# iamsonderr/icl-mixed-precision-gmres

Measured on AMD Instinct MI355X. Metric: GMRES iterations/sec + SpMV achieved HBM GB/s, 10M-nnz CSR, 1/2/4/8 GPUs, higher is better.
Workload: dtype f32; 1 GPU; BAND banded CSR n=1000000, offsets -5..+4, nnz=9999975 (1e6 rows = 10M nnz per GPU, 1 GPU(s)); GMRES(30) mixed (fp32 Arnoldi, f32 accumulation, fp64 residual/update), cgs, identity preconditioner, tol=0; step=one restart cycle = 30 iterations, rows_per_gpu=1000000, nnz=9999975, parallelism=one GPU

## Files before the change

### icl-mixed-precision-gmres_amd/__init__.py

```python
from __future__ import annotations

import ctypes as C
import os
import subprocess
from dataclasses import dataclass, field
from pathlib import Path
from typing import Optional

import numpy as np

from ._abi import (ACCUMS, ENGINES, MODES, ORTHS, PRECS, SPMV_FORMATS, STATUS, CondestResult, HostCsr, RankLayout, SolveArgs, SolveResult,
                   condest_args, condest_dict)

PKG_DIR = Path(__file__).resolve().parent
REPO_DIR = PKG_DIR.parent
LIB_DIR = PKG_DIR / "lib"
HIP_LIB = LIB_DIR / "libmpgmres_hip.so"
HOST_LIB = LIB_DIR / "libmpgmres_host.so"
CLI = PKG_DIR / "bin" / "gmres_perf_test"


def build(jobs: int = 8) -> None:
    subprocess.run(["make", "-C", str(PKG_DIR), f"-j{jobs}"], check=True)

# ... 132 lines not shown
    lib.mpg_halo_local_cols.argtypes = [C.c_void_p, P32]
    lib.mpg_halo_free.argtypes = [C.c_void_p]
    lib.mpg_halo_free.restype = None
    lib.mpg_rccl_unique_id.argtypes = [C.c_char_p, C.c_int]
    lib.mpg_engine_create_dist.argtypes = [C.POINTER(SolveArgs), C.c_void_p, C.c_char_p, _I32, _I32,
                                           C.POINTER(C.c_void_p), C.c_char_p, C.c_int]
    lib.mpg_solve_loopback.argtypes = [C.POINTER(SolveArgs), _I32, C.POINTER(SolveResult)]
    lib.mpg_solve_loopback_ex.argtypes = [C.POINTER(SolveArgs), _I32, C.POINTER(SolveResult), C.c_void_p]
    lib.mpg_solve_multi_gpu.argtypes = [C.POINTER(SolveArgs), _I32, C.c_void_p, C.POINTER(SolveResult), C.c_void_p]
    lib.mpg_engine_comm_ranks.argtypes = [C.c_void_p]
    lib.mpg_engine_sell_columns.argtypes = [C.c_void_p, C.POINTER(C.c_int32), C.POINTER(C.c_int64),
                                            C.POINTER(C.c_int64)]
    lib.mpg_engine_half_stats.argtypes = [C.c_void_p, C.POINTER(C.c_int64)]
    lib.mpg_engine_slices_per_wave.argtypes = [C.c_void_p]
    lib.mpg_engine_givens_folded.argtypes = [C.c_void_p]
    lib.mpg_engine_accum.argtypes = [C.c_void_p]
    lib.mpg_engine_prologue_format.argtypes = [C.c_void_p]
    lib.mpg_engine_sell_shared_slices.argtypes = [C.c_void_p]
    lib.mpg_engine_sell_shared_slices.restype = C.c_int64
    lib.mpg_engine_sell_sigma.argtypes = [C.c_void_p]


_HIP_DECLS = {
    "mpg_error_string": ([C.c_int], C.c_char_p),
    "mpg_ctx_last_error": ([_P], C.c_char_p),
    "mpg_ctx_create": ([C.c_int, C.POINTER(_P)], C.c_int),
    "mpg_ctx_destroy": ([_P], C.c_int),
    "mpg_ctx_sync": ([_P], C.c_int),
    "mpg_ctx_stream": ([_P], _P),
    "mpg_malloc": ([_P, C.c_size_t, C.POINTER(_P)], C.c_int),
# ... 578 lines not shown
        per = (C.c_double * cap)()
        which = {"spmv": 0, "cgs_update": 2, "dots": 3}[phase]
        cnt = self._lib.mpg_engine_time_phase_stamps(self._h, which, reps, C.byref(ms), per, cap)
        if cnt < 0:
            msg = self._lib.mpg_engine_last_error(self._h).decode(errors="replace")
            raise RuntimeError(f"mpg_engine_time_phase_stamps failed ({cnt}): {msg}")
        return ms.value, [per[i] for i in range(min(cnt, cap))]

    def phase_bytes(self, phase: str) -> float:
        return float(self._lib.mpg_engine_phase_bytes(self._h, self.PHASES[phase]))

    def spmv_layout(self) -> dict:
        f, w, cb, st, win = C.c_int32(), C.c_int32(), C.c_int32(), C.c_int64(), C.c_int32()
        if self._lib.mpg_engine_spmv_layout(self._h, C.byref(f), C.byref(w), C.byref(cb), C.byref(st), C.byref(win)):
            raise RuntimeError("mpg_engine_spmv_layout failed")
        return {"format": {1: "csr", 2: "sell", 3: "node"}[f.value], "vec_width": w.value, "col_bytes": cb.value,
                "stored": st.value, "window": bool(win.value),
                "slices_per_wave": int(self._lib.mpg_engine_slices_per_wave(self._h)),
                "givens_folded": bool(self._lib.mpg_engine_givens_folded(self._h) == 1),
                "accum": {0: "f64", 1: "f32"}[int(self._lib.mpg_engine_accum(self._h))],
                "prologue": {1: "csr", 2: "sell", 3: "node"}[int(self._lib.mpg_engine_prologue_format(self._h))]}

    def sell_columns(self) -> dict:
        f, e, i = C.c_int32(), C.c_int64(), C.c_int64()
        if self._lib.mpg_engine_sell_columns(self._h, C.byref(f), C.byref(e), C.byref(i)):
            raise RuntimeError("mpg_engine_sell_columns failed")
        return {"form": {-1: "none", 0: "int32", 1: "int16", 2: "stepped"}[f.value], "csr_slices": e.value,
                "implicit_slices": i.value,
                "shared_slices": int(self._lib.mpg_engine_sell_shared_slices(self._h)),
                "sigma": int(self._lib.mpg_engine_sell_sigma(self._h))}

    def comm_ranks(self) -> int:
        return int(self._lib.mpg_engine_comm_ranks(self._h))

    def half_stats(self) -> dict:
        st = (C.c_int64 * 4)()
# ... 15 lines not shown
```

### icl-mixed-precision-gmres_amd/csrc/arnoldi.hip

```cpp
#include "arnoldi_kernels.hpp"
#include "arnoldi_launch.hpp"

#include <cstdlib>
#include <new>
#include <algorithm>
#include <vector>

using namespace mpg;

namespace {

int64_t sell_copy_bytes(const mpg_arnoldi* a);

void node_prologue_build(mpg_arnoldi* a) {
    const char* e = std::getenv("MPG_NODE_PROLOGUE");
    if ((e && *e == '0') || a->node.nblk == 0 || a->d.n_front != 0 || a->d.outer_type != MPG_F64) return;
    if (hipMalloc((void**)&a->rsum, (size_t)std::max(a->d.n, 1) * sizeof(double)) != hipSuccess) {
        (void)hipGetLastError();
        return;
    }
    if (a->d.val_outer == a->d.val_inner && a->d.inner_val == MPG_F64) {
        a->node_res = &a->node;
        return;
    }
// ... 288 lines not shown
    });
    if (st) return st;
    MPG_LAUNCH_CHECK(a->ctx);
    return MPG_OK;
}

int mpg_arnoldi_reduce(mpg_arnoldi_t a, int ncols) {
    return a && a->acc32 ? mpg_acc32::reduce(a, ncols) : reduce_run<double>(a, ncols);
}

int mpg_arnoldi_spmv(mpg_arnoldi_t a, int k) { return spmv_impl(a, k, 0); }
int mpg_arnoldi_spmv_dots(mpg_arnoldi_t a, int k, int fold) {
    if (fold < 0 || fold > 2) return MPG_ERR_ARG;
    return spmv_impl(a, k, fold, true);
}
int mpg_arnoldi_givens_spmv(mpg_arnoldi_t a, int k) { return spmv_impl(a, k, 1); }
int mpg_arnoldi_givens_partials_spmv(mpg_arnoldi_t a, int k) { return spmv_impl(a, k, 2); }
int mpg_arnoldi_fold_max_m(void) { return kFoldMaxM; }
int mpg_arnoldi_partials_max_cols(void) { return kWideMax; }

constexpr int kFoldMaxGroups = 4096;
int mpg_arnoldi_fold_pays(mpg_arnoldi_t a) {
    if (!a) return 0;
    const char* env = std::getenv("MPG_FOLD_MAX_GROUPS");
    const int64_t limit = env && *env ? std::atoll(env) : kFoldMaxGroups;
    if (a->node.nblk > 0) {
        const int tpw = node_tpw(a->node);
        return (a->node.ntiles + tpw - 1) / tpw <= limit ? 1 : 0;
    }
    const SellCopy& S = a->sell;
// ... 78 lines not shown
```

### icl-mixed-precision-gmres_amd/csrc/arnoldi_acc32.hip

```cpp
#include "arnoldi_launch.hpp"

namespace mpg_acc32 {
int reduce(mpg_arnoldi* a, int ncols) { return reduce_run<float>(a, ncols); }
int spmv(mpg_arnoldi* a, int k, int fold, bool dots) { return spmv_run<float>(a, k, fold, dots); }
int dots(mpg_arnoldi* a, int k, bool combine) { return dots_run<float>(a, k, combine); }
int cgs(mpg_arnoldi* a, int k, int pass, bool givens, bool from_partials, bool no_next) {
    return cgs_run<float>(a, k, pass, givens, from_partials, no_next);
}
int mgs(mpg_arnoldi* a, int k, int j, bool from_partials) { return mgs_run<float>(a, k, j, from_partials); }
int givens(mpg_arnoldi* a, int k, bool from_partials) { return givens_run<float>(a, k, from_partials); }
int update(mpg_arnoldi* a, int k) { return update_run<float>(a, k); }
}
```

### icl-mixed-precision-gmres_amd/csrc/arnoldi_kernels.hpp

```cpp
#pragma once

#include "csr_tile.hpp"
#include "node_tile.hpp"
#include "sell_tile.hpp"
#include "handoff.hpp"
#include "panel.hpp"
#include "internal.hpp"
#include "mpgmres/arnoldi.h"

#include <cstdlib>
#include <new>
#include <algorithm>
#include <vector>

using namespace mpg;

namespace {

constexpr int kNC = 32;
constexpr int kGroups = 1024;
constexpr int kCombineBlock = 1024;
constexpr int kCombineGroups = 256;
constexpr int kOrthMGS = 1, kOrthCGSR = 2;

// ... 854 lines not shown
            }
        }
    }
    for (int i = n4 + blockIdx.x * BS + threadIdx.x; i < n; i += gridDim.x * BS) {
        const A wi = (A)w[i];
#pragma unroll
        for (int c = 0; c < kNC; ++c)
            if (c < nc) acc[c] += (A)Vb[(int64_t)c * ld + i] * wi;
    }
    store_partials<kNC, BS, COMBINE>(acc, nc, partial + (size_t)c0 * gridDim.x);
    if constexpr (COMBINE) {
        if (last_arriver(cnt)) combine_columns<BS, A>(partial, gridDim.x, nc, sums);
    }
}

template <class T, int BS, int NC, class A = double>
__device__ __forceinline__ void dots_panel(int n, const T* __restrict__ V, int64_t ld, const T* __restrict__ w,
                                           double* __restrict__ partial) {
    static_assert(NC >= 1 && NC <= kNC, "one panel");
    constexpr int NP = Pow2Ceil<NC>::v;
    constexpr int B = kColBatch<T>;
    A acc[NP];
#pragma unroll
    for (int c = 0; c < NP; ++c) acc[c] = A(0);
    const int n4 = n & ~3;
    for (int i = 4 * (blockIdx.x * BS + threadIdx.x); i < n4; i += 4 * gridDim.x * BS) {
        A wv[4];
        Row4<T>::load(w + i, wv);
#pragma unroll
        for (int c0 = 0; c0 < NC; c0 += B) {
            Raw4<T> v[B];
#pragma unroll
            for (int u = 0; u < B; ++u)
                if (c0 + u < NC) v[u].load(V + (int64_t)(c0 + u) * ld + i);
            __builtin_amdgcn_sched_barrier(0);
#pragma unroll
            for (int u = 0; u < B; ++u)
                if (c0 + u < NC)
                    acc[c0 + u] += v[u].template at<A>(0) * wv[0] + v[u].template at<A>(1) * wv[1] +
                                   v[u].template at<A>(2) * wv[2] + v[u].template at<A>(3) * wv[3];
            asm volatile("" : "+v"(acc[c0]) : : "memory");
        }
    }
    for (int i = n4 + blockIdx.x * BS + threadIdx.x; i < n; i += gridDim.x * BS) {
        const A wi = (A)w[i];
#pragma unroll
        for (int c = 0; c < NC; ++c) acc[c] += (A)V[(int64_t)c * ld + i] * wi;
    }
    store_partials<NP, BS>(acc, NC, partial);
}

template <class T, int BS, int NC, bool STAMP = false, class A = double>
__global__ __launch_bounds__(BS) void k_dots_nc(int n, const T* __restrict__ V, int64_t ld,
                                                const T* __restrict__ w, double* __restrict__ partial,
                                                unsigned long long* stamp) {
    stamp_at<STAMP>(stamp, 0);
    dots_panel<T, BS, NC, A>(n, V, ld, w, partial);
    stamp_at<STAMP>(stamp, 1);
}

template <class T, int BS, int NCL, class A = double>
__global__ __launch_bounds__(BS) void k_dots_panels(int n, const T* __restrict__ V, int64_t ld,
                                                    const T* __restrict__ w, double* __restrict__ partial) {
    const int c0 = blockIdx.y * kNC;
    double* __restrict__ part = partial + (size_t)c0 * gridDim.x;
    if (blockIdx.y + 1 < gridDim.y) dots_panel<T, BS, kNC, A>(n, V + (int64_t)c0 * ld, ld, w, part);
    else dots_panel<T, BS, NCL, A>(n, V + (int64_t)c0 * ld, ld, w, part);
}

template <class T, int BS, int NC, bool FROM_PARTS = false, bool NEXT_DOTS = false, bool PF = false,
          bool STAMP = false, class A = double>
__global__ __launch_bounds__(BS) void k_cgs_update_nc(int n, const T* __restrict__ V, int64_t ld,
                                                      const double* __restrict__ sums, int part_G,
// ... 587 lines not shown
    double* dpart = nullptr;
    double* sums = nullptr;
    double* report = nullptr;
    unsigned* counters = nullptr;
    int Gd = 1;
    SellCopy sell;
    SellCopy sell_outer;
    NodeCopy node;
    NodeCopy node_outer;
    const NodeCopy* node_res = nullptr;
    double* rsum = nullptr;
    bool outer_is_inner = false;
    double* fd_part = nullptr;
    unsigned* fd_cnt = nullptr;
    int fd_gs = 0, fd_ng = 0;
    bool acc32 = false;

    char* small_at(int slot) const { return static_cast<char*>(small) + (size_t)slot * (d.m + 1) * tsize; }
    void* cs() const { return small_at(0); }
    void* sn() const { return small_at(1); }
    void* s() const { return small_at(2); }
    void* corr() const { return small_at(3); }
    void* inv() const { return small_at(4); }
};

namespace {

int combo_of(const mpg_arnoldi_desc& d) {
    if (d.vec_type == MPG_F64 && d.outer_type == MPG_F64 && d.inner_val == MPG_F64)
        return d.prec_type == MPG_F64 ? 0 : (d.prec_type == MPG_F32 ? 1 : -1);
// ... 50 lines not shown
```

### icl-mixed-precision-gmres_amd/csrc/arnoldi_launch.hpp

```cpp
#pragma once

#include "arnoldi_kernels.hpp"

#include <algorithm>
#include <cstdlib>
#include <type_traits>

namespace {

template <class A, class F>
int dispatch_acc(int combo, F&& f) {
    if constexpr (std::is_same_v<A, double>) {
        return dispatch(combo, f);
    } else {
        switch (combo) {
            case 2: return f(float(), float(), float(), float());
            case 3: return f(float(), double(), float(), float());
            case 4: return f(float(), double(), float(), half_v());
            default: return MPG_ERR_UNSUPPORTED;
        }
    }
}

template <class A>
// ... 142 lines not shown
            Acsr->blocks, Acsr->nblocks, Acsr->rowptr, Acsr->col, static_cast<const VI*>(a->d.val_inner), Acsr->nnz,
            static_cast<const T*>(a->w[k & 1]), static_cast<const T*>(a->inv()), static_cast<T*>(a->V), a->ld, k,
            diag, static_cast<T*>(a->w[(k + 1) & 1]), gf, a->d.inner_row_exp);
        return (int)MPG_OK;
    });
    if (st) return st;
    if (dots) {
        a->last_G = a->fd_ng;
        a->last_part = a->dpart;
    }
    MPG_LAUNCH_CHECK(a->ctx);
    return MPG_OK;
}


inline int wide_groups(const mpg_arnoldi* a, int ncols) {
    const int np = (ncols + kNC - 1) / kNC;
    return std::max(1, std::min(a->Gd, kCombineGroups / np));
}

inline unsigned long long* take_stamp(mpg_arnoldi* a, int64_t waves) {
    unsigned long long* p = a->ctx->stamp_next;
    a->ctx->stamp_next = nullptr;
    return p && waves <= a->ctx->stamp_cap ? p : nullptr;
}

template <class A>
int dots_run(mpg_arnoldi_t a, int k, bool combine) {
    if (!a || k < 0 || k >= a->d.m) return MPG_ERR_ARG;
    const int ndots_all = a->d.orth == kOrthMGS ? 1 : k + 1;
// ... 206 lines not shown
                static_cast<X*>(a->d.x));
        }
        return (int)MPG_OK;
    });
    if (st) return st;
    MPG_LAUNCH_CHECK(a->ctx);
    return MPG_OK;
}


}

namespace mpg_acc32 {
int reduce(mpg_arnoldi* a, int ncols);
int spmv(mpg_arnoldi* a, int k, int fold, bool dots);
int dots(mpg_arnoldi* a, int k, bool combine);
int cgs(mpg_arnoldi* a, int k, int pass, bool givens, bool from_partials, bool no_next);
int mgs(mpg_arnoldi* a, int k, int j, bool from_partials);
int givens(mpg_arnoldi* a, int k, bool from_partials);
int update(mpg_arnoldi* a, int k);
}
```

### icl-mixed-precision-gmres_amd/host/fused_gmres.cpp

```cpp
#include "fused_gmres.hpp"

#include <algorithm>
#include <chrono>
#include <cmath>
#include <cstdio>
#include <cstring>
#include <functional>
#include <stdexcept>
#include <thread>

#include "gmres.hpp"
#include "types_hip.hpp"

namespace mpg {

DevMem::DevMem(mpg_ctx_t c, size_t b) : ctx(c), bytes(b) { check(mpg_malloc(c, b, &p), "mpg_malloc", c); }
DevMem::~DevMem() {
    if (p) mpg_free(ctx, p);
}
DevMem& DevMem::operator=(DevMem&& o) noexcept {
    if (this != &o) {
        if (p) mpg_free(ctx, p);
        ctx = o.ctx;
        p = o.p;
// ... 37 lines not shown
    std::function<double(size_t)> step_loss;
    LostOrthogonalityFused(double tol, double restart_tol, size_t m, size_t max_restarts)
        : Base(tol, m, max_restarts), restart_tol_squared_(restart_tol * restart_tol) {}
    iteration_action check_initial(double r, double nrm, double pr, double pb) override {
        current_loss_squared_ = 0;
        return Base::check_initial(r, nrm, pr, pb);
    }
    iteration_action check(size_t k, double res, double bnorm) override {
        const iteration_action a = Base::check(k, res, bnorm);
        if (a != iteration_next) return a;
        current_loss_squared_ += step_loss(k);
        return current_loss_squared_ >= restart_tol_squared_ ? iteration_restart : iteration_next;
    }
    bool needs_arnoldi_residual() const override { return true; }
};

}

struct FusedEngine::Impl {
    mpg_ctx_t ctx = nullptr;
    mpg_solve_args args{};
    Comm* comm = nullptr;
    ModeTypes ty{};
    int n = 0, n_ext = 0, m = 0, orth = 0;
    int front = 0;
    void* xp = nullptr;
    int64_t nnz = 0;
    DevMem rowptr, col, val64, val_outer_own, val_inner_own, diag, b, x, tmp_t, tmp_p, scal;
    DevMem row_exp;
    int64_t half_stats[4] = {0, 0, 0, 0};
// ... 4 lines not shown
    double* rep[2] = {nullptr, nullptr};
    double* report_host = nullptr;
    int report_len = 0;
    bool pipeline = true;
    DevMem x_snap;
    hipEvent_t report_ev[2] = {nullptr, nullptr};
    hipGraph_t graph = nullptr;
    hipGraphExec_t graph_exec = nullptr;
    bool use_graph = true;
    bool fold = false;
    bool combine = false;
    bool cgs_partials = false;
    bool fuse_dots = false;
    bool fuse_dots_required = false;
    int fuse_dots_k0 = 32;
    int timed = -1;
    bool timed_inplace = false;
    bool timed_graph = false;
    std::vector<hipEvent_t> marks;
    unsigned long long* stamps = nullptr;
    int dup_phase = -1;
    int64_t dup_count = 0;
    int64_t dup_with_dots = 0;
    int64_t stamp_cap = 0, stamp_q = 0, stamp_max = 0;
    std::vector<int32_t> rowptr_host;
    mpg_ilu_t ilu = nullptr;
    bool orthloss = false;
    DevMem loss_S, loss_u;

    ~Impl() {
// ... 222 lines not shown
    conv_->total_iters = 0;
    breakdown.stop = a.stop_on_breakdown != 0;

    const char* env = std::getenv("MPG_NO_GRAPH");
    I.use_graph = !(env && *env == '1') && (!comm || comm->capturable());
    const char* cenv = std::getenv("MPG_COMBINE");
    I.combine = !comm && cenv && *cenv == '1' && I.orth != MPG_ORTH_MGS && I.m <= mpg_arnoldi_fold_max_m();
    const char* penv = std::getenv("MPG_CGS_PARTIALS");
    I.cgs_partials = !I.combine && I.orth != MPG_ORTH_MGS &&
                     (I.orth == MPG_ORTH_CGSR ? (penv && *penv == '1') : !(penv && *penv == '0'));
    const char* denv = std::getenv("MPG_FUSE_DOTS");
    I.fuse_dots = I.cgs_partials && I.orth == MPG_ORTH_CGS && denv && (*denv == '1' || *denv == '2');
    I.fuse_dots_required = I.fuse_dots && *denv == '2';
    const char* kenv = std::getenv("MPG_FUSE_DOTS_K0");
    I.fuse_dots_k0 = kenv && *kenv ? std::max(0, std::min(32, std::atoi(kenv))) : 32;
    const char* fenv = std::getenv("MPG_FOLD_GIVENS");
    bool fold_on = fenv && *fenv ? *fenv != '0' : mpg_arnoldi_fold_pays(I.arn) != 0;
    if (comm && !(fenv && *fenv)) {
        double* flag = I.scal.as<double>() + 6;
        const double no = fold_on ? 0.0 : 1.0;
        check(mpg_memcpy_h2d(ctx, flag, &no, sizeof no), "h2d", ctx);
        comm->allreduce_max(flag, 1, I.stream());
        double any_no = 0;
        check(mpg_memcpy_d2h(ctx, &any_no, flag, sizeof any_no), "d2h", ctx);
        fold_on = any_no == 0.0;
    }
    I.fold = !I.combine && fold_on && I.m <= mpg_arnoldi_fold_max_m();
    check(mpg_ctx_sync(ctx), "sync", ctx);
    setup_seconds = std::chrono::duration<double>(clk::now() - t0).count();
    prologue();
// ... 47 lines not shown

void FusedEngine::step(int k, bool fold) {
    Impl& I = *p_;
    if (I.fuse_dots && !I.comm && !I.ilu && I.orth == MPG_ORTH_CGS && I.cgs_partials && !I.combine &&
        k + 1 <= I.fuse_dots_k0) {
        timed(0, [&] { check(mpg_arnoldi_spmv(I.arn, k), "spmv", I.ctx); });
        const int st = mpg_arnoldi_spmv_dots(I.arn, k, fold && k > 0 ? 2 : 0);
        timed_end(0);
        if (st == MPG_OK) {
            check(mpg_arnoldi_cgs_partials(I.arn, k), "cgs", I.ctx);
            if (!fold) givens(k);
            return;
        }
        if (st != MPG_ERR_UNSUPPORTED || I.fuse_dots_required) check(st, "spmv+dots", I.ctx);
        I.fuse_dots = false;
    }
    if (fold && k > 0) {
        if (I.comm)
            I.comm->allreduce_sum_and_halo(mpg_arnoldi_partials_dev(I.arn), mpg_arnoldi_partials_count(I.arn),
                                           mpg_arnoldi_wprev_dev(I.arn, k), mpg_arnoldi_vec_bytes(I.arn),
                                           I.stream());
        timed(0, [&] { check(mpg_arnoldi_spmv(I.arn, k), "spmv", I.ctx); });
        check(mpg_arnoldi_givens_partials_spmv(I.arn, k), "givens+spmv", I.ctx);
        dup(0, [&] { check(mpg_arnoldi_givens_partials_spmv(I.arn, k), "givens+spmv", I.ctx); });
        timed_end(0);
    } else {
        if (I.comm) I.comm->halo(mpg_arnoldi_wprev_dev(I.arn, k), mpg_arnoldi_vec_bytes(I.arn), I.stream());
        timed(0, [&] { check(mpg_arnoldi_spmv(I.arn, k), "spmv", I.ctx); });
        check(mpg_arnoldi_spmv(I.arn, k), "spmv", I.ctx);
        dup(0, [&] { check(mpg_arnoldi_spmv(I.arn, k), "spmv", I.ctx); });
// ... 365 lines not shown
}

double FusedEngine::phase_bytes(int which) const {
    const Impl& I = *p_;
    const double n = I.n, z = (double)I.nnz, sT = (double)dsize(I.ty.T), sX = (double)dsize(I.ty.X);
    const double sV = (double)dsize(I.ty.VI), sP = (double)dsize(I.ty.P);
    const double jac = I.args.prec == MPG_PREC_JACOBI ? 1.0 : 0.0;
    if (which == 0) {
        return z * (sV + 4) + (n + 1) * 4 + 2 * n * sT + jac * n * sP;
    }
    if (which == 1) return z * (sX + 4) + (n + 1) * 4 + 3 * n * sX + n * sT + jac * n * sP;
    if (which == 4) {
        int32_t fmt = 0, W = 0, cb = 0, win = 0;
        int64_t stored = 0;
        check(mpg_arnoldi_spmv_layout(I.arn, &fmt, &W, &cb, &stored, &win), "layout", I.ctx);
        const double vec = 3 * n * sT + jac * n * sP;
        if (fmt == 2 || fmt == 3) return (double)mpg_arnoldi_sell_matrix_bytes(I.arn) + vec;
        return z * (sV + 4) + (n + 1) * 4 + vec;
    }
    if (which == 3) {
        double cols = 0;
        for (int k = 0; k < I.m; ++k) cols += (I.orth == MPG_ORTH_MGS ? 1 : k + 1);
        return (cols / I.m + 1) * n * sT;
    }
    return ((I.m - 1) / 2.0 + 1) * n * sT + 2 * n * sT;
}

mpg_arnoldi_t FusedEngine::arnoldi() const { return p_->arn; }
const int64_t* FusedEngine::half_stats() const { return p_->half_stats; }
bool FusedEngine::givens_folded() const { return p_->fold; }

constexpr int kTimedReplays = 10;

double FusedEngine::time_phase(int which, int reps, bool inplace, std::vector<double>* per_launch) {
    measured = true;
    Impl& I = *p_;
    if (inplace && which != 0) throw std::invalid_argument("in-place timing covers the Arnoldi SpMV only");
    I.timed = which;
    I.timed_inplace = inplace;
    I.marks.clear();
    for (int r = 0; r < reps; ++r) cycle_program();
    I.timed = -1;
    I.timed_inplace = false;
    hipck(hipStreamSynchronize(I.stream()), "sync");
    float total_ms = 0;
// ... 194 lines not shown
    cleanup();
    if (!count) throw StatusError(MPG_ERR_UNSUPPORTED, "no launch of the phase stored stamps");
    return total / count;
}

double FusedEngine::time_phase_dup(int which, int reps, int64_t* launches) {
    measured = true;
    Impl& I = *p_;
    if (!I.use_graph) throw StatusError(MPG_ERR_UNSUPPORTED, "the cycle is not captured (MPG_NO_GRAPH / eager ranks)");
    if (which != 0 && which != 2 && which != 3) throw std::invalid_argument("phase: 0 spmv, 2 cgs update, 3 dots");
    hipGraph_t g[2] = {nullptr, nullptr};
    hipGraphExec_t ge[2] = {nullptr, nullptr};
    hipEvent_t ev[2] = {nullptr, nullptr};
    auto cleanup = [&] {
        I.dup_phase = -1;
        for (int q = 0; q < 2; ++q) {
            if (ge[q]) (void)hipGraphExecDestroy(ge[q]);
            if (g[q]) (void)hipGraphDestroy(g[q]);
            if (ev[q]) (void)hipEventDestroy(ev[q]);
        }
    };
    std::vector<double> diff;
    int64_t added = 0, with_dots = 0;
    try {
        for (int q = 0; q < 2; ++q) {
            I.dup_phase = q ? which : -1;
            I.dup_count = 0;
            I.dup_with_dots = 0;
            hipck(hipStreamBeginCapture(I.stream(), hipStreamCaptureModeThreadLocal), "begin capture");
            try {
                cycle_program();
            } catch (...) {
                (void)hipStreamEndCapture(I.stream(), &g[q]);
                throw;
            }
            hipck(hipStreamEndCapture(I.stream(), &g[q]), "end capture");
            hipck(hipGraphInstantiate(&ge[q], g[q], nullptr, nullptr, 0), "instantiate");
            if (q) {
                added = I.dup_count;
                with_dots = I.dup_with_dots;
            }
        }
        I.dup_phase = -1;
        if (added < 1) throw StatusError(MPG_ERR_UNSUPPORTED, "the cycle has no launch of that phase");
        for (hipEvent_t& e : ev) hipck(hipEventCreate(&e), "event");
        for (int q = 0; q < 2; ++q) hipck(hipGraphLaunch(ge[q], I.stream()), "graph launch");
        hipck(hipStreamSynchronize(I.stream()), "sync");
        for (int r = 0; r < reps; ++r) {
            float ms[2] = {0, 0};
            for (int q = 0; q < 2; ++q) {
                hipck(hipEventRecord(ev[0], I.stream()), "record");
                hipck(hipGraphLaunch(ge[q], I.stream()), "graph launch");
                hipck(hipEventRecord(ev[1], I.stream()), "record");
                hipck(hipEventSynchronize(ev[1]), "sync");
                hipck(hipEventElapsedTime(&ms[q], ev[0], ev[1]), "elapsed");
            }
            diff.push_back((double)(ms[1] - ms[0]) / (double)added);
        }
    } catch (...) {
        cleanup();
        (void)hipGetLastError();
        throw;
    }
    cleanup();
    if (launches) *launches = added;
    std::sort(diff.begin(), diff.end());
    double ms = diff[diff.size() / 2];
    if (with_dots) ms -= time_phase_dup(3, reps) * (double)with_dots / (double)added;
    return ms;
}

void fill_history(const FusedEngine& e, mpg_solve_result* r) {
    r->status = e.status;
    r->restarts = e.restarts;
    r->inner_k = e.inner_k;
    r->total_iters = (int64_t)e.total_iters();
    r->minvb_norm = e.minvb_norm;
    r->setup_seconds = e.setup_seconds;
    r->n_cycles = (int64_t)e.cycles.size();
    for (size_t c = 0; c < e.cycles.size() && (int64_t)c < r->cycle_cap; ++c) {
        if (r->cyc_r_norm) r->cyc_r_norm[c] = e.cycles[c].r_norm;
        if (r->cyc_normalization) r->cyc_normalization[c] = e.cycles[c].normalization;
        if (r->cyc_beta) r->cyc_beta[c] = e.cycles[c].beta;
// ... 194 lines not shown
int mpg_engine_accum(mpg_engine_t e) {
    if (!e || !e->eng) return MPG_ERR_ARG;
    return mpg_arnoldi_accum(e->eng->arnoldi());
}

int mpg_engine_prologue_format(mpg_engine_t e) {
    if (!e || !e->eng) return MPG_ERR_ARG;
    return mpg_arnoldi_prologue_format(e->eng->arnoldi());
}

int mpg_engine_givens_folded(mpg_engine_t e) {
    if (!e || !e->eng) return MPG_ERR_ARG;
    return e->eng->givens_folded() ? 1 : 0;
}

int mpg_engine_comm_ranks(mpg_engine_t e) {
    if (!e || !e->eng) return MPG_ERR_ARG;
    return e->comm ? e->comm->transport_ranks() : 1;
}

int64_t mpg_engine_sell_shared_slices(mpg_engine_t e) {
    if (!e || !e->eng) return MPG_ERR_ARG;
    return mpg_arnoldi_sell_shared_slices(e->eng->arnoldi());
}

int mpg_engine_sell_sigma(mpg_engine_t e) {
    if (!e || !e->eng) return MPG_ERR_ARG;
    return mpg_arnoldi_sell_sigma(e->eng->arnoldi());
}

// ... 27 lines not shown
```

### icl-mixed-precision-gmres_amd/host/fused_gmres.hpp

```cpp
#ifndef MPGMRES_FUSED_GMRES_HPP
#define MPGMRES_FUSED_GMRES_HPP

#include <hip/hip_runtime.h>

#include <memory>
#include <string>
#include <vector>

#include "IterUtil.hpp"
#include "mpgmres/arnoldi.h"
#include "mpgmres/capi.h"
#include "mpgmres/solve.h"

namespace mpg {

class Comm {
public:
    virtual ~Comm() {}
    virtual int size() const = 0;
    virtual int rank() const = 0;
    virtual void allreduce_sum(double* dev, int count, hipStream_t s) = 0;
    virtual void allreduce_max(double* dev, int count, hipStream_t s) = 0;
    virtual void halo(void* dev_vec, int elem_bytes, hipStream_t s) = 0;
    virtual void allreduce_sum_and_halo(double* dev, int count, void* dev_vec, int elem_bytes, hipStream_t s) {
// ... 27 lines not shown
    FusedEngine(mpg_ctx_t ctx, const mpg_solve_args& args, Comm* comm = nullptr, int n_ext = -1, int n_front = 0);
    ~FusedEngine();

    int run(int max_cycles, bool& done);
    void finish_report(mpg_solve_result* r);

    size_t total_iters() const { return conv_->total_iterations(); }
    double time_phase(int which, int reps, bool inplace = false, std::vector<double>* per_launch = nullptr);
    double time_phase_graph(int which, int reps, std::vector<double>* per_launch = nullptr);
    double time_phase_stamps(int which, int reps, std::vector<double>* per_launch = nullptr);
    double time_phase_dup(int which, int reps, int64_t* launches = nullptr);
    double phase_bytes(int which) const;
    mpg_arnoldi_t arnoldi() const;
    const int64_t* half_stats() const;
    bool givens_folded() const;
    void sync();

    std::vector<CycleRecord> cycles;
    std::vector<double> step_res;
    std::vector<int> step_cycle;
    int status = 0;
    int64_t restarts = 0;
    int64_t inner_k = 0;
    double minvb_norm = 0, b_norm = 0, a_norm = 0;
    double setup_seconds = 0;
    BreakdownLog breakdown;
    bool measured = false;

private:
    struct Impl;
// ... 39 lines not shown
```

### include/mpgmres/arnoldi.h

```cpp
#ifndef MPGMRES_ARNOLDI_H
#define MPGMRES_ARNOLDI_H

#include <stdint.h>

#include "mpgmres/capi.h"

#ifdef __cplusplus
extern "C" {
#endif

typedef enum { MPG_F64 = 0, MPG_F32 = 1, MPG_F16 = 2 } mpg_dtype_t;

typedef struct mpg_arnoldi* mpg_arnoldi_t;

typedef struct {
    int32_t n;
    int32_t n_ext;
    int32_t m;
    int32_t orth;
    int32_t vec_type;
    int32_t outer_type;
    int32_t prec_type;
    int32_t inner_val;
    int32_t jacobi;
// ... 28 lines not shown
int mpg_arnoldi_spmv(mpg_arnoldi_t a, int k);
int mpg_arnoldi_dots(mpg_arnoldi_t a, int k);
int mpg_arnoldi_cgs(mpg_arnoldi_t a, int k, int pass);
int mpg_arnoldi_cgs_partials(mpg_arnoldi_t a, int k);
int mpg_arnoldi_partials_max_cols(void);
int mpg_arnoldi_cgsr_wide_pass(mpg_arnoldi_t a, int k, int pass);
int mpg_arnoldi_mgs(mpg_arnoldi_t a, int k, int j);
int mpg_arnoldi_mgs_partials(mpg_arnoldi_t a, int k, int j);
int mpg_arnoldi_givens(mpg_arnoldi_t a, int k);
int mpg_arnoldi_givens_partials(mpg_arnoldi_t a, int k);
int mpg_arnoldi_givens_spmv(mpg_arnoldi_t a, int k);
int mpg_arnoldi_dots_sums(mpg_arnoldi_t a, int k);
int mpg_arnoldi_cgs_givens(mpg_arnoldi_t a, int k, int pass);
int mpg_arnoldi_givens_partials_spmv(mpg_arnoldi_t a, int k);
int mpg_arnoldi_spmv_dots(mpg_arnoldi_t a, int k, int fold);
int mpg_arnoldi_fold_max_m(void);
int mpg_arnoldi_fold_pays(mpg_arnoldi_t a);
int mpg_arnoldi_update(mpg_arnoldi_t a, int k);
int mpg_arnoldi_reduce(mpg_arnoldi_t a, int ncols);

double* mpg_arnoldi_sums_dev(mpg_arnoldi_t a);
void* mpg_arnoldi_wprev_dev(mpg_arnoldi_t a, int k);
int mpg_arnoldi_vec_bytes(mpg_arnoldi_t a);
const double* mpg_arnoldi_report_dev(mpg_arnoldi_t a);
int mpg_arnoldi_report_len(mpg_arnoldi_t a);
const void* mpg_arnoldi_basis_dev(mpg_arnoldi_t a, int64_t* ld);
const void* mpg_arnoldi_hessenberg_dev(mpg_arnoldi_t a);
const void* mpg_arnoldi_inv_dev(mpg_arnoldi_t a);
int mpg_arnoldi_time_next_spmv(mpg_arnoldi_t a, void* start_event, void* stop_event);
int mpg_arnoldi_stamp_next(mpg_arnoldi_t a, unsigned long long* slots, int64_t cap_waves);
// ... 20 lines not shown
```

### include/mpgmres/solve.h

```cpp
#ifndef MPGMRES_SOLVE_H
#define MPGMRES_SOLVE_H

#include <stddef.h>
#include <stdint.h>

#ifdef __cplusplus
extern "C" {
#endif

typedef enum {
    MPG_MODE_MIXED = 0,
    MPG_MODE_BASELINE = 1,
    MPG_MODE_SINGLE_PREC = 2,
    MPG_MODE_SINGLE = 3,
    MPG_MODE_MIXED_HALF = 4
} mpg_mode_t;

typedef enum { MPG_ORTH_CGS = 0, MPG_ORTH_MGS = 1, MPG_ORTH_CGSR = 2 } mpg_orth_t;

typedef enum { MPG_PREC_ILU = 0, MPG_PREC_ILU_JACOBI = 1, MPG_PREC_JACOBI = 2, MPG_PREC_IDENTITY = 3 } mpg_prec_t;

typedef enum {
    MPG_ENGINE_SURFACE = 0,
    MPG_ENGINE_FUSED = 1
// ... 61 lines not shown
int mpg_engine_report(mpg_engine_t e, mpg_solve_result* result);
int mpg_engine_time_phase(mpg_engine_t e, int which, int reps, double* avg_ms);
int mpg_engine_time_spmv_incycle(mpg_engine_t e, int cycles, double* avg_ms, double* per_launch_ms, int cap);
int mpg_engine_time_phase_dup(mpg_engine_t e, int which, int reps, double* avg_ms, int64_t* launches);
int mpg_engine_time_phase_stamps(mpg_engine_t e, int which, int reps, double* avg_ms, double* per_launch_ms,
                                 int cap);
int mpg_engine_time_phase_graph(mpg_engine_t e, int which, int reps, double* avg_ms, double* per_launch_ms,
                                int cap);
double mpg_engine_phase_bytes(mpg_engine_t e, int which);
int mpg_engine_spmv_layout(mpg_engine_t e, int32_t* format, int32_t* vec_width, int32_t* col_bytes,
                           int64_t* stored, int32_t* window);
int mpg_engine_sell_columns(mpg_engine_t e, int32_t* form, int64_t* csr_slices, int64_t* implicit_slices);
int64_t mpg_engine_sell_shared_slices(mpg_engine_t e);
int mpg_engine_sell_sigma(mpg_engine_t e);
int mpg_engine_givens_folded(mpg_engine_t e);
int mpg_engine_accum(mpg_engine_t e);
int mpg_engine_prologue_format(mpg_engine_t e);
int mpg_engine_comm_ranks(mpg_engine_t e);
int mpg_engine_slices_per_wave(mpg_engine_t e);
int mpg_engine_half_stats(mpg_engine_t e, int64_t* stats);
int mpg_engine_destroy(mpg_engine_t e);

int mpg_cycle_program_counts(int64_t* recorded, int64_t* replayed, int64_t* voided);
int mpg_surface_ride_counts(int64_t* redirects, int64_t* rides, int64_t* flushed);
int mpg_surface_spmv_counts(int64_t* node, int64_t* sell, int64_t* csr);
int mpg_surface_host_norm_hits(int64_t* hits);
int mpg_surface_host_norm_pairs(int64_t* pairs);

#ifdef __cplusplus
}
// ... 3 lines not shown
```

Baseline: 27130 GMRES iterations/s.

## Fuse SELL SpMV with CGS dot products in one windowed launch per step

Adds a k_step_dots kernel that computes the banded SELL SpMV from an LDS window, writes the normalized basis vector and new w, then immediately computes the CGS dot products against the basis using the w and newest-column values staged in LDS. Some leading basis columns are held in registers. The host selects this path per step, by default only within a k range and only when single GPU, CGS with partials, and uniform int16 SELL. The aim is to drop a separate dots launch and avoid re-reading w and v_k from HBM, at the cost of a larger kernel with more LDS and register pressure.

```diff
diff --git a/icl-mixed-precision-gmres_amd/__init__.py b/icl-mixed-precision-gmres_amd/__init__.py
--- a/icl-mixed-precision-gmres_amd/__init__.py
+++ b/icl-mixed-precision-gmres_amd/__init__.py
@@ -170,6 +170,8 @@
     lib.mpg_engine_half_stats.argtypes = [C.c_void_p, C.POINTER(C.c_int64)]
     lib.mpg_engine_slices_per_wave.argtypes = [C.c_void_p]
     lib.mpg_engine_givens_folded.argtypes = [C.c_void_p]
+    lib.mpg_engine_step_dots_steps.argtypes = [C.c_void_p]
+    lib.mpg_engine_step_dots_status.argtypes = [C.c_void_p, C.c_int]
     lib.mpg_engine_accum.argtypes = [C.c_void_p]
     lib.mpg_engine_prologue_format.argtypes = [C.c_void_p]
     lib.mpg_engine_sell_shared_slices.argtypes = [C.c_void_p]
@@ -778,12 +780,16 @@
         f, w, cb, st, win = C.c_int32(), C.c_int32(), C.c_int32(), C.c_int64(), C.c_int32()
         if self._lib.mpg_engine_spmv_layout(self._h, C.byref(f), C.byref(w), C.byref(cb), C.byref(st), C.byref(win)):
             raise RuntimeError("mpg_engine_spmv_layout failed")
-        return {"format": {1: "csr", 2: "sell", 3: "node"}[f.value], "vec_width": w.value, "col_bytes": cb.value,
+        fused = int(self._lib.mpg_engine_step_dots_steps(self._h))
+        return {**({"dots_fused": fused} if fused > 0 else {}), "format": {1: "csr", 2: "sell", 3: "node"}[f.value], "vec_width": w.value, "col_bytes": cb.value,
                 "stored": st.value, "window": bool(win.value),
                 "slices_per_wave": int(self._lib.mpg_engine_slices_per_wave(self._h)),
                 "givens_folded": bool(self._lib.mpg_engine_givens_folded(self._h) == 1),
                 "accum": {0: "f64", 1: "f32"}[int(self._lib.mpg_engine_accum(self._h))],
                 "prologue": {1: "csr", 2: "sell", 3: "node"}[int(self._lib.mpg_engine_prologue_format(self._h))]}
+
+    def step_dots_status(self, k: int) -> int:
+        return int(self._lib.mpg_engine_step_dots_status(self._h, k))
 
     def sell_columns(self) -> dict:
         f, e, i = C.c_int32(), C.c_int64(), C.c_int64()
diff --git a/icl-mixed-precision-gmres_amd/csrc/arnoldi.hip b/icl-mixed-precision-gmres_amd/csrc/arnoldi.hip
--- a/icl-mixed-precision-gmres_amd/csrc/arnoldi.hip
+++ b/icl-mixed-precision-gmres_amd/csrc/arnoldi.hip
@@ -326,6 +326,12 @@
     if (fold < 0 || fold > 2) return MPG_ERR_ARG;
     return spmv_impl(a, k, fold, true);
 }
+int mpg_arnoldi_step_dots(mpg_arnoldi_t a, int k, int fold) {
+    return a && a->acc32 ? mpg_acc32::step_dots(a, k, fold) : step_dots_run<double>(a, k, fold);
+}
+int mpg_arnoldi_step_dots_supported(mpg_arnoldi_t a, int k) {
+    return a && a->acc32 ? mpg_acc32::step_dots_ok(a, k) : step_dots_check<double>(a, k);
+}
 int mpg_arnoldi_givens_spmv(mpg_arnoldi_t a, int k) { return spmv_impl(a, k, 1); }
 int mpg_arnoldi_givens_partials_spmv(mpg_arnoldi_t a, int k) { return spmv_impl(a, k, 2); }
 int mpg_arnoldi_fold_max_m(void) { return kFoldMaxM; }
diff --git a/icl-mixed-precision-gmres_amd/csrc/arnoldi_acc32.hip b/icl-mixed-precision-gmres_amd/csrc/arnoldi_acc32.hip
--- a/icl-mixed-precision-gmres_amd/csrc/arnoldi_acc32.hip
+++ b/icl-mixed-precision-gmres_amd/csrc/arnoldi_acc32.hip
@@ -3,6 +3,8 @@
 namespace mpg_acc32 {
 int reduce(mpg_arnoldi* a, int ncols) { return reduce_run<float>(a, ncols); }
 int spmv(mpg_arnoldi* a, int k, int fold, bool dots) { return spmv_run<float>(a, k, fold, dots); }
+int step_dots(mpg_arnoldi* a, int k, int fold) { return step_dots_run<float>(a, k, fold); }
+int step_dots_ok(const mpg_arnoldi* a, int k) { return step_dots_check<float>(a, k); }
 int dots(mpg_arnoldi* a, int k, bool combine) { return dots_run<float>(a, k, combine); }
 int cgs(mpg_arnoldi* a, int k, int pass, bool givens, bool from_partials, bool no_next) {
     return cgs_run<float>(a, k, pass, givens, from_partials, no_next);
diff --git a/icl-mixed-precision-gmres_amd/csrc/arnoldi_kernels.hpp b/icl-mixed-precision-gmres_amd/csrc/arnoldi_kernels.hpp
--- a/icl-mixed-precision-gmres_amd/csrc/arnoldi_kernels.hpp
+++ b/icl-mixed-precision-gmres_amd/csrc/arnoldi_kernels.hpp
@@ -892,8 +892,18 @@
     }
 }
 
-template <class T, int BS, int NC, class A = double>
-__device__ __forceinline__ void dots_panel(int n, const T* __restrict__ V, int64_t ld, const T* __restrict__ w,
+template <class T, class A>
+struct DotsGlobal {
+    static constexpr bool kStaged = false;
+    static constexpr int kHeld = 0;
+    const T* __restrict__ w;
+    Raw4<T> held[1];
+    __device__ __forceinline__ void load_w(int i, A (&wv)[4]) const { Row4<T>::load(w + i, wv); }
+    __device__ __forceinline__ Raw4<T> newest(int) const { return Raw4<T>(); }
+};
+
+template <class T, int BS, int NC, class A = double, class SRC>
+__device__ __forceinline__ void dots_panel_from(int n, const T* __restrict__ V, int64_t ld, const SRC& src,
                                            double* __restrict__ partial) {
     static_assert(NC >= 1 && NC <= kNC, "one panel");
     constexpr int NP = Pow2Ceil<NC>::v;
@@ -902,15 +912,20 @@
 #pragma unroll
     for (int c = 0; c < NP; ++c) acc[c] = A(0);
     const int n4 = n & ~3;
+    bool first = SRC::kHeld > 0;
     for (int i = 4 * (blockIdx.x * BS + threadIdx.x); i < n4; i += 4 * gridDim.x * BS) {
         A wv[4];
-        Row4<T>::load(w + i, wv);
+        src.load_w(i, wv);
 #pragma unroll
         for (int c0 = 0; c0 < NC; c0 += B) {
             Raw4<T> v[B];
 #pragma unroll
             for (int u = 0; u < B; ++u)
-                if (c0 + u < NC) v[u].load(V + (int64_t)(c0 + u) * ld + i);
+                if (c0 + u < NC) {
+                    if (SRC::kStaged && c0 + u == NC - 1) v[u] = src.newest(i);
+                    else if (c0 + u < SRC::kHeld && first) v[u] = src.held[c0 + u < SRC::kHeld ? c0 + u : 0];
+                    else v[u].load(V + (int64_t)(c0 + u) * ld + i);
+                }
             __builtin_amdgcn_sched_barrier(0);
 #pragma unroll
             for (int u = 0; u < B; ++u)
@@ -919,13 +934,22 @@
                                    v[u].template at<A>(2) * wv[2] + v[u].template at<A>(3) * wv[3];
             asm volatile("" : "+v"(acc[c0]) : : "memory");
         }
-    }
-    for (int i = n4 + blockIdx.x * BS + threadIdx.x; i < n; i += gridDim.x * BS) {
-        const A wi = (A)w[i];
-#pragma unroll
-        for (int c = 0; c < NC; ++c) acc[c] += (A)V[(int64_t)c * ld + i] * wi;
+        if constexpr (SRC::kHeld > 0) first = false;
+    }
+    if constexpr (!SRC::kStaged) {
+        for (int i = n4 + blockIdx.x * BS + threadIdx.x; i < n; i += gridDim.x * BS) {
+            const A wi = (A)src.w[i];
+#pragma unroll
+            for (int c = 0; c < NC; ++c) acc[c] += (A)V[(int64_t)c * ld + i] * wi;
+        }
     }
     store_partials<NP, BS>(acc, NC, partial);
+}
+
+template <class T, int BS, int NC, class A = double>
+__device__ __forceinline__ void dots_panel(int n, const T* __restrict__ V, int64_t ld, const T* __restrict__ w,
+                                           double* __restrict__ partial) {
+    dots_panel_from<T, BS, NC, A>(n, V, ld, DotsGlobal<T, A>{w, {}}, partial);
 }
 
 template <class T, int BS, int NC, bool STAMP = false, class A = double>
@@ -935,6 +959,154 @@
     stamp_at<STAMP>(stamp, 0);
     dots_panel<T, BS, NC, A>(n, V, ld, w, partial);
     stamp_at<STAMP>(stamp, 1);
+}
+
+constexpr int kStepDotsRows = 4 * kCombineBlock;
+
+template <class T, class A, int HELD>
+struct DotsStaged {
+    static constexpr bool kStaged = true;
+    static constexpr int kHeld = HELD;
+    const T* wst;
+    const T* vkst;
+    int base;
+    Raw4<T> held[HELD > 0 ? HELD : 1];
+    __device__ __forceinline__ void load_w(int i, A (&wv)[4]) const { Row4<T>::load(wst + (i - base), wv); }
+    __device__ __forceinline__ Raw4<T> newest(int i) const {
+        Raw4<T> r;
+        r.load(vkst + (i - base));
+        return r;
+    }
+};
+
+template <class T, class P, int W, bool FOLD, int BE, int NC, bool PF, class A>
+__global__ __launch_bounds__(kCombineBlock) void k_step_dots(int n, int nslices, const int16_t* __restrict__ col,
+                                                             const T* __restrict__ val, const T* __restrict__ wprev,
+                                                             const T* __restrict__ inv_p, T* __restrict__ V,
+                                                             int64_t ld, int k, const P* __restrict__ diag,
+                                                             T* __restrict__ w, GivensFold<T> fold,
+                                                             const int32_t* __restrict__ spat,
+                                                             const int64_t* __restrict__ coff,
+                                                             const int16_t* __restrict__ pat, int64_t ustride,
+                                                             double* __restrict__ dpart) {
+    static_assert(std::is_same_v<T, float>, "fp32 basis and values");
+    using CI = int16_t;
+    using Row = SellRow<T, CI, W, (MPG_SELL_NT != 0), BE>;
+    constexpr int BS = kCombineBlock, SPW = 4;
+    constexpr int RB = kStepDotsRows, WL = kWinLo + RB + kWinHi;
+    static_assert(SPW * (BS / kWave) * kWave == RB, "four slices per wave cover the workgroup's rows");
+    __shared__ __attribute__((aligned(16))) T win[WL];
+    __shared__ __attribute__((aligned(16))) T wst[RB];
+    const int tid = threadIdx.x, lane = tid & (kWave - 1), wid = wave_id();
+    const int base = (int)blockIdx.x * RB;
+    const int s0 = (int)blockIdx.x * (RB / kWave) + wid * SPW;
+    Row row[SPW];
+    bool live_p[SPW];
+#pragma unroll
+    for (int p = 0; p < SPW; ++p) {
+        live_p[p] = s0 + p < nslices;
+        row[p].init_uniform(live_p[p] ? s0 + p : 0, ustride, spat, coff);
+    }
+    __builtin_amdgcn_sched_barrier(0);
+    A part = A(0);
+    if constexpr (FOLD) {
+        part = (A)fold.norm2[tid < fold.nparts ? tid : 0];
+        if (tid >= fold.nparts) part = A(0);
+    }
+    __builtin_amdgcn_sched_barrier(0);
+    const int i4 = base + 4 * tid;
+    const bool in4 = i4 < n;
+    Raw4<T> wr;
+    wr.load(wprev + (in4 ? i4 : 0));
+    const int hc = tid < kWinLo ? base - kWinLo + tid : base + RB + (tid - kWinLo);
+    const bool hin = tid < kWinLo + kWinHi && hc >= 0 && hc < n;
+    const T wh = wprev[hin ? hc : 0];
+    __builtin_amdgcn_sched_barrier(0);
+#pragma unroll
+    for (int p = 0; p < SPW; ++p) {
+        row[p].init_vals(lane, val);
+        row[p].load_vals(0);
+    }
+    __builtin_amdgcn_sched_barrier(0);
+#pragma unroll
+    for (int p = 0; p < SPW; ++p) {
+        row[p].init_finish(lane, col, val, nullptr, pat);
+        row[p].load_cols(0);
+    }
+    __builtin_amdgcn_sched_barrier(0);
+    constexpr int B = kColBatch<T>;
+    constexpr int HMAX = FOLD ? 6 : B;
+    constexpr int HELD = !PF ? 0 : NC - 1 < HMAX ? NC - 1 : HMAX;
+    DotsStaged<T, A, HELD> src;
+    src.wst = wst;
+    src.vkst = win + kWinLo;
+    src.base = base;
+    if constexpr (HELD > 0) {
+#pragma unroll
+        for (int u = 0; u < HELD; ++u) src.held[u].load(V + (int64_t)u * ld + (in4 ? i4 : 0));
+    }
+    __builtin_amdgcn_sched_barrier(0);
+    T inv;
+    double nrm2sq = 0.0;
+    if constexpr (FOLD) {
+        constexpr int NG = kBlock / kWave;
+        __shared__ A scratch[NG];
+        __shared__ T inv_s;
+        if (fold.nparts > 0) {
+            if (wid < NG) {
+                const A v = wave_sum(part + A(0));
+                if (lane == 0) scratch[wid] = v;
+            }
+            lds_barrier();
+            A r = A(0);
+#pragma unroll
+            for (int q = 0; q < NG; ++q) r += scratch[q];
+            nrm2sq = (double)r;
+        } else {
+            nrm2sq = fold.norm2[0];
+        }
+        if (tid == 0) inv_s = inv_of_norm2<T>(nrm2sq);
+        lds_barrier();
+        inv = inv_s;
+    } else {
+        inv = *inv_p;
+    }
+    {
+        T vq[4];
+#pragma unroll
+        for (int r = 0; r < 4; ++r) vq[r] = in4 ? (T)(wr.template at<T>(r) * inv) : T(0);
+        Row4<T>::store(win + kWinLo + 4 * tid, vq);
+        if (tid < kWinLo + kWinHi) win[tid < kWinLo ? tid : RB + tid] = hin ? (T)(wh * inv) : T(0);
+    }
+    lds_barrier();
+    auto xv = [&](int c) { return (double)win[c - base + kWinLo]; };
+    A sum[SPW] = {};
+#pragma unroll
+    for (int p = 0; p < SPW; ++p)
+        if (live_p[p]) row[p].sum(0, xv, sum[p]);
+#pragma unroll
+    for (int p = 0; p < SPW; ++p) {
+        if (live_p[p])
+            for (int q = Row::U; q < row[p].steps; q += Row::U) {
+                row[p].load(q);
+                row[p].sum(q, xv, sum[p]);
+            }
+        const int i = (s0 + p) * kWave + lane;
+        T wi = T(0);
+        if (live_p[p] && i < n) {
+            const T t = (T)sum[p];
+            wi = precond<T, P>(t, diag, i);
+            w[i] = wi;
+            V[(int64_t)k * ld + i] = win[i - base + kWinLo];
+        }
+        wst[i - base] = wi;
+    }
+    lds_barrier();
+    dots_panel_from<T, BS, NC, A>(n, V, ld, src, dpart);
+    if constexpr (FOLD) {
+        __shared__ T col_s[kFoldMaxM + 2], c_s[kFoldMaxM + 2], s_s[kFoldMaxM + 2];
+        if (blockIdx.x == 0) givens_block(fold.g, nrm2sq, col_s, c_s, s_s);
+    }
 }
 
 template <class T, int BS, int NCL, class A = double>
@@ -1552,6 +1724,8 @@
     double* fd_part = nullptr;
     unsigned* fd_cnt = nullptr;
     int fd_gs = 0, fd_ng = 0;
+    int sd_k = -1, sd_G = 0;
+    double* sd_part = nullptr;
     bool acc32 = false;
 
     char* small_at(int slot) const { return static_cast<char*>(small) + (size_t)slot * (d.m + 1) * tsize; }
diff --git a/icl-mixed-precision-gmres_amd/csrc/arnoldi_launch.hpp b/icl-mixed-precision-gmres_amd/csrc/arnoldi_launch.hpp
--- a/icl-mixed-precision-gmres_amd/csrc/arnoldi_launch.hpp
+++ b/icl-mixed-precision-gmres_amd/csrc/arnoldi_launch.hpp
@@ -180,6 +180,61 @@
 }
 
 
+template <class A>
+int step_dots_check(const mpg_arnoldi* a, int k) {
+    if (!a || k < 0 || k >= a->d.m) return MPG_ERR_ARG;
+    const SellCopy& S = a->sell;
+    const bool ok = std::is_same_v<A, float> && (a->combo == 2 || a->combo == 3) &&
+                    a->d.orth != kOrthMGS && a->d.orth != kOrthCGSR && k + 1 <= kNC &&
+                    a->d.n > 0 && a->d.n % 4 == 0 &&
+                    (int64_t)a->Gd * kStepDotsRows >= a->d.n &&
+                    a->front == 0 && a->d.n_ext == a->d.n &&
+                    S.nslices > 0 && S.c16 && S.win && !S.rows && sell_uniform(S) && S.W == 2 &&
+                    S.ustride / kWave <= 10;
+    return ok ? MPG_OK : MPG_ERR_UNSUPPORTED;
+}
+
+template <class A>
+int step_dots_run(mpg_arnoldi_t a, int k, int fold) {
+    if (!a || k < 0 || k >= a->d.m || fold < 0 || fold > 2) return MPG_ERR_ARG;
+    if (int st = step_dots_check<A>(a, k)) return st;
+    if (fold && (k < 1 || a->d.m > kFoldMaxM)) return MPG_ERR_ARG;
+    if constexpr (std::is_same_v<A, float>) {
+        using T = float;
+        using P = float;
+        const bool again = fold == 2 && a->sd_k == k && a->last_part == a->dpart;
+        if (fold == 2 && !again) {
+            a->sd_k = k;
+            a->sd_part = a->last_part;
+            a->sd_G = a->last_G;
+        }
+        if (fold == 2 && (a->sd_G > kBlock || a->sd_part == a->dpart)) return MPG_ERR_ARG;
+        GivensFold<T> gf{nullptr, 0, {}};
+        if (fold) gf = GivensFold<T>{fold == 2 ? a->sd_part : a->sums, fold == 2 ? a->sd_G : 0, givens_args<T>(a, k - 1)};
+        const SellCopy& S = a->sell;
+        const P* diag = a->d.jacobi ? static_cast<const P*>(a->d.diag) : nullptr;
+        int st = with_nc<kNC>(k + 1, [&](auto nc) {
+            constexpr int NC = decltype(nc)::value;
+            auto go = [&](auto kern) {
+                launch_timed(a->ctx, kern, dim3(a->Gd), dim3(kCombineBlock), a->d.n, S.nslices,
+                             static_cast<const int16_t*>(S.col), static_cast<const T*>(S.val),
+                             static_cast<const T*>(a->w[k & 1]), static_cast<const T*>(a->inv()),
+                             static_cast<T*>(a->V), a->ld, k, diag, static_cast<T*>(a->w[(k + 1) & 1]), gf, S.spat,
+                             S.coff, static_cast<const int16_t*>(S.pat), S.ustride, a->dpart);
+                return (int)MPG_OK;
+            };
+            return fold ? go(k_step_dots<T, P, 2, true, 10, NC, true, A>) : go(k_step_dots<T, P, 2, false, 10, NC, true, A>);
+        });
+        if (st) return st;
+        a->last_G = a->Gd;
+        a->last_part = a->dpart;
+        MPG_LAUNCH_CHECK(a->ctx);
+        return MPG_OK;
+    } else {
+        return MPG_ERR_UNSUPPORTED;
+    }
+}
+
 inline int wide_groups(const mpg_arnoldi* a, int ncols) {
     const int np = (ncols + kNC - 1) / kNC;
     return std::max(1, std::min(a->Gd, kCombineGroups / np));
@@ -416,6 +471,8 @@
 namespace mpg_acc32 {
 int reduce(mpg_arnoldi* a, int ncols);
 int spmv(mpg_arnoldi* a, int k, int fold, bool dots);
+int step_dots(mpg_arnoldi* a, int k, int fold);
+int step_dots_ok(const mpg_arnoldi* a, int k);
 int dots(mpg_arnoldi* a, int k, bool combine);
 int cgs(mpg_arnoldi* a, int k, int pass, bool givens, bool from_partials, bool no_next);
 int mgs(mpg_arnoldi* a, int k, int j, bool from_partials);
diff --git a/icl-mixed-precision-gmres_amd/host/fused_gmres.cpp b/icl-mixed-precision-gmres_amd/host/fused_gmres.cpp
--- a/icl-mixed-precision-gmres_amd/host/fused_gmres.cpp
+++ b/icl-mixed-precision-gmres_amd/host/fused_gmres.cpp
@@ -75,6 +75,8 @@
     }
     bool needs_arnoldi_residual() const override { return true; }
 };
+
+constexpr int kStepDotsLo = 1, kStepDotsHi = 32;
 
 }
 
@@ -109,6 +111,24 @@
     bool fuse_dots = false;
     bool fuse_dots_required = false;
     int fuse_dots_k0 = 32;
+    int step_dots = 0;
+    int step_dots_lo = 1, step_dots_hi = 0;
+    int64_t dup_with_step = 0;
+    bool dup_step_only = false;
+
+    bool step_dots_engine_ok() const { return !(comm || ilu || orth != MPG_ORTH_CGS || !cgs_partials || combine); }
+    bool step_dots_at(int k) const {
+        if (step_dots == 0) return false;
+        if (step_dots == 2) return true;
+        if (!step_dots_engine_ok()) return false;
+        if (step_dots < 0 && (k + 1 < step_dots_lo || k + 1 > step_dots_hi)) return false;
+        return mpg_arnoldi_step_dots_supported(arn, k) == MPG_OK;
+    }
+    int step_dots_steps() const {
+        int c = 0;
+        for (int k = 0; k < m; ++k) c += step_dots_at(k) && mpg_arnoldi_step_dots_supported(arn, k) == MPG_OK;
+        return c;
+    }
     int timed = -1;
     bool timed_inplace = false;
     bool timed_graph = false;
@@ -361,6 +381,14 @@
     I.fuse_dots_required = I.fuse_dots && *denv == '2';
     const char* kenv = std::getenv("MPG_FUSE_DOTS_K0");
     I.fuse_dots_k0 = kenv && *kenv ? std::max(0, std::min(32, std::atoi(kenv))) : 32;
+    {
+        const char* senv = std::getenv("MPG_STEP_DOTS");
+        I.step_dots = senv && *senv >= '0' && *senv <= '2' ? *senv - '0' : -1;
+        const char* lo = std::getenv("MPG_STEP_DOTS_LO");
+        const char* hi = std::getenv("MPG_STEP_DOTS_HI");
+        I.step_dots_lo = lo && *lo ? std::atoi(lo) : kStepDotsLo;
+        I.step_dots_hi = hi && *hi ? std::atoi(hi) : kStepDotsHi;
+    }
     const char* fenv = std::getenv("MPG_FOLD_GIVENS");
     bool fold_on = fenv && *fenv ? *fenv != '0' : mpg_arnoldi_fold_pays(I.arn) != 0;
     if (comm && !(fenv && *fenv)) {
@@ -438,6 +466,37 @@
         }
         if (st != MPG_ERR_UNSUPPORTED || I.fuse_dots_required) check(st, "spmv+dots", I.ctx);
         I.fuse_dots = false;
+    }
+    if (I.step_dots_at(k)) {
+        const int f = fold && k > 0 ? 2 : 0;
+        if (!I.step_dots_engine_ok())
+            throw StatusError(MPG_ERR_UNSUPPORTED, "MPG_STEP_DOTS=2: the SpMV + dots launch needs one GPU and plain CGS "
+                                                   "with in-launch sums, without ILU");
+        timed(0, [&] { check(mpg_arnoldi_spmv(I.arn, k), "spmv", I.ctx); });
+        const int st = mpg_arnoldi_step_dots(I.arn, k, f);
+        if (st == MPG_OK) {
+            dup(0, [&] { check(mpg_arnoldi_step_dots(I.arn, k, f), "spmv+dots", I.ctx); });
+            timed_end(0);
+            timed(2, [&] { check(mpg_arnoldi_cgs_partials(I.arn, k), "cgs", I.ctx); });
+            check(mpg_arnoldi_cgs_partials(I.arn, k), "cgs", I.ctx);
+            dup(2, [&] {
+                check(mpg_arnoldi_step_dots(I.arn, k, f), "spmv+dots", I.ctx);
+                check(mpg_arnoldi_cgs_partials(I.arn, k), "cgs", I.ctx);
+                ++I.dup_with_step;
+            });
+            timed_end(2);
+            if (!fold) givens(k);
+            return;
+        }
+        timed_end(0);
+        check(st, "spmv+dots", I.ctx);
+    }
+    if (I.dup_step_only && I.dup_phase == 0) {
+        const int keep = I.dup_phase;
+        I.dup_phase = -1;
+        step(k, fold);
+        I.dup_phase = keep;
+        return;
     }
     if (fold && k > 0) {
         if (I.comm)
@@ -833,14 +892,21 @@
         int32_t fmt = 0, W = 0, cb = 0, win = 0;
         int64_t stored = 0;
         check(mpg_arnoldi_spmv_layout(I.arn, &fmt, &W, &cb, &stored, &win), "layout", I.ctx);
-        const double vec = 3 * n * sT + jac * n * sP;
+        double cols = 0;
+        for (int k = 0; k < I.m; ++k)
+            if (I.step_dots_at(k)) cols += k;
+        const double vec = 3 * n * sT + jac * n * sP + cols / I.m * n * sT;
         if (fmt == 2 || fmt == 3) return (double)mpg_arnoldi_sell_matrix_bytes(I.arn) + vec;
         return z * (sV + 4) + (n + 1) * 4 + vec;
     }
     if (which == 3) {
-        double cols = 0;
-        for (int k = 0; k < I.m; ++k) cols += (I.orth == MPG_ORTH_MGS ? 1 : k + 1);
-        return (cols / I.m + 1) * n * sT;
+        double cols = 0, launches = 0;
+        for (int k = 0; k < I.m; ++k)
+            if (!I.step_dots_at(k)) {
+                cols += (I.orth == MPG_ORTH_MGS ? 1 : k + 1);
+                launches += 1;
+            }
+        return (cols / I.m + launches / I.m) * n * sT;
     }
     return ((I.m - 1) / 2.0 + 1) * n * sT + 2 * n * sT;
 }
@@ -848,6 +914,8 @@
 mpg_arnoldi_t FusedEngine::arnoldi() const { return p_->arn; }
 const int64_t* FusedEngine::half_stats() const { return p_->half_stats; }
 bool FusedEngine::givens_folded() const { return p_->fold; }
+int FusedEngine::step_dots_steps() const { return p_->step_dots_steps(); }
+int FusedEngine::step_dots_status(int k) const { return mpg_arnoldi_step_dots_supported(p_->arn, k); }
 
 constexpr int kTimedReplays = 10;
 
@@ -1072,6 +1140,7 @@
     hipEvent_t ev[2] = {nullptr, nullptr};
     auto cleanup = [&] {
         I.dup_phase = -1;
+        I.dup_step_only = false;
         for (int q = 0; q < 2; ++q) {
             if (ge[q]) (void)hipGraphExecDestroy(ge[q]);
             if (g[q]) (void)hipGraphDestroy(g[q]);
@@ -1079,12 +1148,16 @@
         }
     };
     std::vector<double> diff;
-    int64_t added = 0, with_dots = 0;
+    int64_t added = 0, with_dots = 0, with_step = 0;
+    const bool step_only = I.dup_step_only;
+    I.dup_step_only = false;
     try {
         for (int q = 0; q < 2; ++q) {
             I.dup_phase = q ? which : -1;
+            I.dup_step_only = q && step_only;
             I.dup_count = 0;
             I.dup_with_dots = 0;
+            I.dup_with_step = 0;
             hipck(hipStreamBeginCapture(I.stream(), hipStreamCaptureModeThreadLocal), "begin capture");
             try {
                 cycle_program();
@@ -1097,9 +1170,11 @@
             if (q) {
                 added = I.dup_count;
                 with_dots = I.dup_with_dots;
+                with_step = I.dup_with_step;
             }
         }
         I.dup_phase = -1;
+        I.dup_step_only = false;
         if (added < 1) throw StatusError(MPG_ERR_UNSUPPORTED, "the cycle has no launch of that phase");
         for (hipEvent_t& e : ev) hipck(hipEventCreate(&e), "event");
         for (int q = 0; q < 2; ++q) hipck(hipGraphLaunch(ge[q], I.stream()), "graph launch");
@@ -1125,6 +1200,10 @@
     std::sort(diff.begin(), diff.end());
     double ms = diff[diff.size() / 2];
     if (with_dots) ms -= time_phase_dup(3, reps) * (double)with_dots / (double)added;
+    if (with_step) {
+        I.dup_step_only = true;
+        ms -= time_phase_dup(0, reps) * (double)with_step / (double)added;
+    }
     return ms;
 }
 
@@ -1349,6 +1428,16 @@
     return e->eng->givens_folded() ? 1 : 0;
 }
 
+int mpg_engine_step_dots_steps(mpg_engine_t e) {
+    if (!e || !e->eng) return MPG_ERR_ARG;
+    return e->eng->step_dots_steps();
+}
+
+int mpg_engine_step_dots_status(mpg_engine_t e, int k) {
+    if (!e || !e->eng) return MPG_ERR_ARG;
+    return e->eng->step_dots_status(k);
+}
+
 int mpg_engine_comm_ranks(mpg_engine_t e) {
     if (!e || !e->eng) return MPG_ERR_ARG;
     return e->comm ? e->comm->transport_ranks() : 1;
diff --git a/icl-mixed-precision-gmres_amd/host/fused_gmres.hpp b/icl-mixed-precision-gmres_amd/host/fused_gmres.hpp
--- a/icl-mixed-precision-gmres_amd/host/fused_gmres.hpp
+++ b/icl-mixed-precision-gmres_amd/host/fused_gmres.hpp
@@ -65,6 +65,8 @@
     mpg_arnoldi_t arnoldi() const;
     const int64_t* half_stats() const;
     bool givens_folded() const;
+    int step_dots_steps() const;
+    int step_dots_status(int k) const;
     void sync();
 
     std::vector<CycleRecord> cycles;
diff --git a/include/mpgmres/arnoldi.h b/include/mpgmres/arnoldi.h
--- a/include/mpgmres/arnoldi.h
+++ b/include/mpgmres/arnoldi.h
@@ -66,6 +66,8 @@
 int mpg_arnoldi_cgs_givens(mpg_arnoldi_t a, int k, int pass);
 int mpg_arnoldi_givens_partials_spmv(mpg_arnoldi_t a, int k);
 int mpg_arnoldi_spmv_dots(mpg_arnoldi_t a, int k, int fold);
+int mpg_arnoldi_step_dots(mpg_arnoldi_t a, int k, int fold);
+int mpg_arnoldi_step_dots_supported(mpg_arnoldi_t a, int k);
 int mpg_arnoldi_fold_max_m(void);
 int mpg_arnoldi_fold_pays(mpg_arnoldi_t a);
 int mpg_arnoldi_update(mpg_arnoldi_t a, int k);
diff --git a/include/mpgmres/solve.h b/include/mpgmres/solve.h
--- a/include/mpgmres/solve.h
+++ b/include/mpgmres/solve.h
@@ -99,6 +99,8 @@
 int64_t mpg_engine_sell_shared_slices(mpg_engine_t e);
 int mpg_engine_sell_sigma(mpg_engine_t e);
 int mpg_engine_givens_folded(mpg_engine_t e);
+int mpg_engine_step_dots_steps(mpg_engine_t e);
+int mpg_engine_step_dots_status(mpg_engine_t e, int k);
 int mpg_engine_accum(mpg_engine_t e);
 int mpg_engine_prologue_format(mpg_engine_t e);
 int mpg_engine_comm_ranks(mpg_engine_t e);
```

Measured after the change: 27660 GMRES iterations/s, median of 6. 1.02x the previous value.
